# LongTarget/Fasim-LongTarget

Measured on AMD Instinct MI355X. Metric: SW Gcells/s (logical, whole job: stage 1+2+3 of the triplex scan), higher is better.
Workload: dtype u8

## Files before the change

### fasim-longtarget_amd/csrc/align.hip

```cpp
#include <hip/hip_runtime.h>
#include <stdint.h>
#include <stdlib.h>
#include "kernels.h"
#include "systolic.h"

namespace fasim {

constexpr int AL_SCALE = 32;
constexpr int AL_NEG = -32768;
constexpr int CODE_VOID = 4;
constexpr int CODE_SN = 5;
constexpr int TAG_LAST = 8;
constexpr int TAG_HZ = 16;
constexpr int FWD_KROW = 0x1FFFF;

__global__ void k_build_stream(const uint8_t* __restrict__ tcodes, const FwdProb* __restrict__ probs, int32_t nprob,
	uint8_t* __restrict__ stream, const uint32_t* __restrict__ zones)
{
	const int p = blockIdx.x;
	if (p >= nprob) return;
	const FwdProb pb = probs[p];
	uint8_t* s = stream + pb.stream_off;
	const uint32_t z = zones ? zones[p] : 0u;
	const int z1 = (int)(z & 0xffu), z2 = (int)((z >> 8) & 0xffu), z3 = (int)((z >> 16) & 0xffu);
// ... 490 lines not shown
			const int gp = in ? A.lo(k) : GL_NEG;
			const int ep = in ? A.hi(k) : GL_NEG;
			int e = max(ep - GAP_EXT, gp - GAP_OPEN);
			int g = diag > GL_NEG / 2 ? diag + swsc(q[read_end - i], tcode) : GL_NEG;
			g = max(g, max(e, F));
			const int rest = min(R - 1 - i, colrest);
			if (g <= 0 || g + 5 * rest < S) g = GL_NEG;
			if (e <= 0 || e + 5 * rest < S) e = GL_NEG;
			if (g == S) { *ref_begin = ref_end - j; *read_begin = read_end - i; return 0; }
			diag = gp;
			A.set(k, g, e);
			if (g > GL_NEG / 2 || e > GL_NEG / 2) { if (nlo < 0) nlo = i; nhi = i; }
			F = max(F - GAP_EXT, g - GAP_OPEN);
			if (F <= 0) F = GL_NEG;
			if (i > hi && F <= GL_NEG / 2 && diag <= GL_NEG / 2) break;
			if (i - lo + 2 >= FL_RING) return 2;
		}
		if (nlo < 0) return 1;
		lo = nlo; hi = nhi;
	}
	return 1;
}

template <int FL_WORDS, int FL_CELLS>
__global__ void __launch_bounds__(64) k_finish_lds(const uint8_t* __restrict__ tcodes, const uint8_t* __restrict__ qcodes,
	const FwdProb* __restrict__ probs, const FwdOut* __restrict__ fwd, const int32_t* __restrict__ order, int32_t nprob,
	uint8_t* __restrict__ dirs, AlignOutDev* __restrict__ out, uint32_t* __restrict__ cigar_pool, uint32_t pool_cap,
	uint32_t* __restrict__ pool_count)
{
	constexpr int FL_RING = FL_WORDS, FL_W = FL_WORDS / 2;
	__shared__ uint32_t lds[FL_WORDS * 64];
	const int gid = blockIdx.x * blockDim.x + threadIdx.x;
	if (gid >= nprob) return;
	const int pi = order ? order[gid] : gid;
	LdsArena A; A.base = lds + threadIdx.x;
	uint8_t* dir = dirs + (int64_t)blockIdx.x * (64 * FL_CELLS) + threadIdx.x;
	const FwdProb pb = probs[pi];
	const FwdOut fo = fwd[pi];
	AlignOutDev* o = out + pi;
	o->sw_score = 0; o->ref_begin = 0; o->ref_end = fo.ref_end; o->query_begin = 0; o->query_end = fo.read_end; o->cigar_len = 0;
	o->cigar_off = 0;
	if (fo.flags & 1) { o->status = 10; return; }
	if (fo.score <= 0 || fo.ref_end < 0) { o->status = 0; return; }
	const uint8_t* tw = tcodes + pb.tbase;
	int ref_begin = fo.ref_begin, read_begin = fo.read_begin;
	if (!(fo.flags & 2)) {
		if (fo.score >= 148 && fo.score < 255 - BIAS) { o->status = 11; return; }
		const int r = reverse_pass_lds<FL_RING>(tw, qcodes, fo.score, fo.ref_end, fo.read_end, A, &ref_begin, &read_begin);
		if (r) { o->status = r == 2 ? 2 : 11; return; }
	}
	o->ref_begin = ref_begin; o->query_begin = read_begin;
	const uint8_t* ref = tw + ref_begin;
	const uint8_t* read = qcodes + read_begin;
	const int refLen = fo.ref_end - ref_begin + 1, readLen = fo.read_end - read_begin + 1, score = fo.score;
	int band = (refLen > readLen ? refLen - readLen : readLen - refLen) + 1;
	int maxv = 0, width = 0, width_d = 0;
	do {
		width = band * 2 + 3; width_d = band * 2 + 1;
		if (width + 1 > FL_W || width_d * readLen > FL_CELLS) { o->status = 2; return; }
		for (int j = 1; j < width - 1; j++) A.set_lo(j, 0);
		for (int i = 0; i < readLen; i++) {
			int beg = 0, end = refLen - 1, u = 0;
			if (i - band > beg) beg = i - band;
			if (i + band < end) end = i + band;
			const int edge = end + 1 < width - 1 ? end + 1 : width - 1;
			int f = 0;
			A.set(0, 0, 0); A.set(edge, 0, 0); A.set_lo(FL_W, 0);
			const int x = i - band > 0 ? i - band : 0;
			const int xp = i - 1 - band > 0 ? i - 1 - band : 0;
			const int rd = read[i];
			const int rowcell = width_d * i;
			for (int j = beg; j <= end; j++) {
				u = j - x + 1;
				const int e = j - xp + 1, b = j - x, d = j - xp;
				int t1 = i == 0 ? -GAP_OPEN : A.lo(e) - GAP_OPEN;
				int t2 = i == 0 ? -GAP_EXT : A.hi(e) - GAP_EXT;
				const int ev = t1 > t2 ? t1 : t2;
				const int de = t1 > t2 ? 1 : 0;
				t1 = A.lo(FL_W + b) - GAP_OPEN;
				t2 = f - GAP_EXT;
				f = t1 > t2 ? t1 : t2;
				const int df = t1 > t2 ? 1 : 0;
				const int e1 = ev > 0 ? ev : 0;
				const int f1 = f > 0 ? f : 0;
				t1 = e1 > f1 ? e1 : f1;
				t2 = A.lo(d) + swsc(ref[j], rd);
				const int hv = t1 > t2 ? t1 : t2;
				A.set_hi(u, ev);
				A.set_lo(FL_W + u, hv);
				if (hv > maxv) maxv = hv;
				const int dh = (t1 <= t2) ? 0 : (e1 > f1 ? 1 : 2);
				dir[(int64_t)(rowcell + (j - x)) * 64] = (uint8_t)(de | (df << 1) | (dh << 2));
			}
			for (int j = 1; j <= u; j++) A.set_lo(j, A.lo(FL_W + j));
		}
		band *= 2;
		if (maxv < score && band > 4 * (refLen + readLen) + 16) { o->status = 3; return; }
	} while (maxv < score);
	band /= 2;
	uint32_t rc[ALIGN_MAX_CIGAR];
	int l = 0;
	int i = readLen - 1, j = refLen - 1, e = 0, state = 2, op = 0, prev_op = 0, status = 0;
	while (i > 0) {
		const int x = i - band > 0 ? i - band : 0;
		int beg = 0, end = refLen - 1;
		if (i - band > beg) beg = i - band;
		if (i + band < end) end = i + band;
		if (j < beg || j > end) { status = 3; break; }
		const uint32_t nib = dir[(int64_t)(width_d * i + (j - x)) * 64];
		int dv;
		const int dE = (nib & 1) ? 3 : 2, dF = (nib & 2) ? 5 : 4;
		if (state == 0) dv = dE; else if (state == 1) dv = dF; else { const int dh = (nib >> 2) & 3; dv = dh == 0 ? 1 : (dh == 1 ? dE : dF); }
		if (dv == 1) { --i; --j; state = 2; op = 0; }
		else if (dv == 2) { --i; state = 0; op = 1; }
		else if (dv == 3) { --i; state = 2; op = 1; }
		else if (dv == 4) { --j; state = 1; op = 2; }
		else { --j; state = 2; op = 2; }
		if (op == prev_op) ++e;
		else {
			if (l >= ALIGN_MAX_CIGAR) { status = 4; break; }
			rc[l++] = cig(e, prev_op);
			prev_op = op; e = 1;
		}
	}
	if (status == 0) {
		if (op == 0) { if (l >= ALIGN_MAX_CIGAR) status = 4; else rc[l++] = cig(e + 1, 0); }
		else { if (l + 2 > ALIGN_MAX_CIGAR) status = 4; else { rc[l++] = cig(e, op); rc[l++] = cig(1, 0); } }
	}
	if (status == 0) {
		const uint32_t off = atomicAdd(pool_count, (uint32_t)l);
		if ((uint64_t)off + (uint64_t)l > (uint64_t)pool_cap) status = 4;
		else { o->cigar_off = off; for (int k = 0; k < l; k++) cigar_pool[off + k] = rc[l - 1 - k]; }
	}
	o->status = status;
	if (status != 0) return;
	o->sw_score = score;
	o->cigar_len = l;
}

hipError_t launch_finish(const uint8_t* tcodes, const uint8_t* qcodes, const FwdProb* probs, const FwdOut* fwd, const int32_t* order,
	int32_t nprob, uint8_t* dirs, AlignOutDev* out, uint32_t* cigar_pool, uint32_t pool_cap, uint32_t* pool_count, hipStream_t st)
{
	if (nprob <= 0) return hipSuccess;
	hipError_t err = hipMemsetAsync(pool_count, 0, sizeof(uint32_t), st);
	if (err != hipSuccess) return err;
	hipLaunchKernelGGL((k_finish_lds<64, 2048>), dim3((nprob + 63) / 64), dim3(64), 0, st, tcodes, qcodes, probs, fwd, order, nprob, dirs, out,
		cigar_pool, pool_cap, pool_count);
	return hipGetLastError();
}

hipError_t launch_finish_mid(const uint8_t* tcodes, const uint8_t* qcodes, const FwdProb* probs, const FwdOut* fwd, const int32_t* idx_list,
	int32_t nlist, uint8_t* dirs, AlignOutDev* out, uint32_t* cigar_pool, uint32_t pool_cap, uint32_t* pool_count, hipStream_t st)
{
	if (nlist <= 0) return hipSuccess;
	static bool attr_set = false;
	if (!attr_set) { (void)hipFuncSetAttribute((const void*)k_finish_lds<256, 16384>, hipFuncAttributeMaxDynamicSharedMemorySize, 64 * 1024); attr_set = true; }
	hipLaunchKernelGGL((k_finish_lds<256, 16384>), dim3((nlist + 63) / 64), dim3(64), 0, st, tcodes, qcodes, probs, fwd, idx_list, nlist, dirs, out,
		cigar_pool, pool_cap, pool_count);
	return hipGetLastError();
}

hipError_t launch_finish_big(const uint8_t* tcodes, const uint8_t* qcodes, const FwdProb* probs, const FwdOut* fwd,
	const int32_t* idx_list, int32_t nlist, uint8_t* scratch, int32_t scratch_cap, AlignOutDev* out, uint32_t* cigar_pool,
	uint32_t pool_cap, uint32_t* pool_count, hipStream_t st)
{
	if (nlist <= 0) return hipSuccess;
	hipLaunchKernelGGL(k_finish, dim3((nlist + 63) / 64), dim3(64), 0, st, tcodes, qcodes, probs, fwd, nlist, scratch, scratch_cap, out,
		cigar_pool, pool_cap, pool_count, idx_list);
	return hipGetLastError();
}

}
```

### fasim-longtarget_amd/csrc/engine.cpp

```cpp
#include "engine.h"

extern "C" {

void fasim_params_default(fasim_params* p)
{
	p->rule = 0; p->cutLength = 5000; p->strand = 0; p->overlapLength = 100; p->ntMin = 20; p->ntMax = 100000;
	p->scoreMin = 0.0f; p->minIdentity = 60.0f; p->minStability = 1.0f; p->penaltyT = -1000; p->penaltyC = 0;
	p->cDistance = 15; p->cLength = 50; p->classicSim = 0;
}

const char* fasim_last_error(const fasim_engine* e) { return e ? e->err.c_str() : g_last_error.c_str(); }

int fasim_engine_create(int device, fasim_engine** out) { return fasim_engine_create_ex(device, 0, out); }

int fasim_engine_create_ex(int device, int32_t flags, fasim_engine** out)
{
	if (!out) return fail(nullptr, FASIM_E_ARG, "null out pointer");
	*out = nullptr;
	const bool tune = !(flags & FASIM_CREATE_NO_PROCESS_TUNING);
	if (tune) setenv("GPU_MAX_HW_QUEUES", "8", 0);
	if (tune) {
		static const bool once = [] {
			const char* e = getenv("FASIM_MALLOPT");
			if (e && atoi(e) == 0) return false;
// ... 25 lines not shown
	const char* env = getenv("FASIM_HOST_THREADS");
	E->host_threads = env ? std::max(1, atoi(env)) : (int)std::min(96u, std::max(1u, hc * 3 / 8));
	E->host_threads_total = E->host_threads;
	E->host_threads_explicit = env != nullptr;
	const char* v1 = getenv("FASIM_SCAN_V1");
	E->scan_v1 = v1 && atoi(v1) != 0;
	const char* a1 = getenv("FASIM_ALIGN_V1");
	E->align_v1 = a1 && atoi(a1) != 0;
	const char* sw = getenv("FASIM_STRIPED_WINDOW");
	E->striped_window = sw && atoi(sw) != 0;
	*out = E;
	return FASIM_OK;
}

void fasim_engine_destroy(fasim_engine* e)
{
	if (!e) return;
	for (fasim_engine* w : e->workers) fasim_engine_destroy(w);
	e->workers.clear();
	(void)hipSetDevice(e->device);
	DevBuf* bufs[] = { &e->q1, &e->q2, &e->enc_lut, &e->counter, &e->dna, &e->seg_start, &e->seg_len, &e->enc_ids, &e->tcodes,
		&e->colmax, &e->probs, &e->max_out, &e->unit_len, &e->stage1, &e->hits, &e->hits_total, &e->hit_off, &e->hit_cnt, &e->thr,
		&e->ends, &e->bprobs, &e->bout, &e->scratch, &e->dna_res, &e->colmax16, &e->unit_ids, &e->flags, &e->stage1_in, &e->hits2,
		&e->fprobs, &e->ftasks, &e->fstream, &e->fout, &e->aout, &e->cigpool, &e->cigcount, &e->forder, &e->scratch2, &e->boundary, &e->fboundary, &e->unit_hz,
		&e->unit_first, &e->hz_cols, &e->hz_plan, &e->hz_base, &e->hz_items, &e->snap, &e->hz_state, &e->hz_rows, &e->hz_chunk, &e->hz_src, &e->hz_zero,
		&e->qsim, &e->sim_min, &e->sim_row, &e->sim_ev, &e->sim_cnt, &e->sim_nodes,
		&e->ublk, &e->btarget, &e->bidx, &e->bcounts, &e->blist[0], &e->blist[1], &e->blist[2], &e->bslots[0], &e->bslots[1], &e->bslots[2],
		&e->bprev, &e->lane_ub, &e->fzones, &e->fubslot, &e->bdec, &e->btab, &e->swin, &e->unit_ovf, &e->track, &e->track_phase, &e->track_sat, &e->track_peaks, &e->sites_counts, &e->sites_offsets, &e->sites_runs, &e->sites_sat, &e->sa_q, &e->sa_tcodes, &e->sa_probs, &e->sa_ends, &e->sa_rows, &e->sa_items, &e->sa_dirs, &e->sa_cigar, &e->sa_ciglen,
		&e->rowmax16, &e->row_out, &e->row_gfirst, &e->row_sat, &e->oligo_q, &e->hist, &e->hist_zone, &e->hist_zones, &e->hist_sat,
		&e->vr_q, &e->vr_dna, &e->vr_alt, &e->vr_wins, &e->vr_probs, &e->vr_tcodes, &e->vr_rows, &e->vr_touch, &e->vr_out };
	for (auto& t : e->timed) { (void)hipEventDestroy(t.a); (void)hipEventDestroy(t.b); }
	for (hipEvent_t ev : e->ev_pool) (void)hipEventDestroy(ev);
	for (DevBuf* b : bufs) b->release();
	if (e->pin_dna) (void)hipHostFree(e->pin_dna);
	if (e->pin_sim) (void)hipHostFree(e->pin_sim);
	if (e->st) (void)hipStreamDestroy(e->st);
	delete e;
}

int fasim_set_option(fasim_engine* E, const char* key, int32_t value)
{
	if (!E || !key) return fail(E, FASIM_E_ARG, "null argument");
	if (!strcmp(key, "workers")) E->opt_workers = value > 0 ? value : 0;
	else if (!strcmp(key, "seg_batch")) E->opt_seg_batch = value > 0 ? value : 0;
	else if (!strcmp(key, "taper")) E->opt_taper = value;
	else if (!strcmp(key, "heavy_gate")) E->opt_gate = value;
	else if (!strcmp(key, "hazard_chunks")) E->hz_chunks = value;
	else if (!strcmp(key, "hazard_snapshots")) E->hz_snap = value;
	else if (!strcmp(key, "hazard_chunk_cols")) E->hz_target = value > 0 ? std::max(64, value) : 0;
	else if (!strcmp(key, "hazard_hot_weight")) E->hz_hot_w = value > 0 ? std::min(32, value) : 0;
	else if (!strcmp(key, "host_threads")) { if (value > 0) { E->host_threads = value; E->host_threads_total = value; E->host_threads_explicit = true; } }
	else if (!strcmp(key, "numa_affinity")) E->opt_numa = value != 0;
	else if (!strcmp(key, "band")) E->opt_band = value;
	else if (!strcmp(key, "dp_f16")) E->opt_dp_f16 = value;
	else if (!strcmp(key, "site_short")) E->opt_site_short = value;
	else if (!strcmp(key, "sim_lds")) E->opt_sim_lds = value < 0 ? -1 : value != 0;
	else if (!strcmp(key, "site_chunk")) E->opt_site_chunk = value > 0 ? value : 0;
	else if (!strcmp(key, "striped_window")) E->striped_window = value > 0;
	else return fail(E, FASIM_E_ARG, "unknown option %s", key);
	return FASIM_OK;
}

static int refuse_long_query(fasim_engine* E, int64_t len, int index)
{
	char which[32] = "";
	if (index >= 0) snprintf(which, sizeof which, " (query %d)", index);
	return fail(E, FASIM_E_UNSUPPORTED, "query of %lld nt%s exceeds the limit of %d nt: above it the reference's 16-bit stage-1 pass "
		"overruns its fixed workspace (stats.h:397) and its output is undefined", (long long)len, which, FASIM_MAX_QUERY);
}

int fasim_set_query(fasim_engine* E, const char* rna, int32_t len)
{
	if (!E) return fail(nullptr, FASIM_E_ARG, "null engine");
	if (!rna || len <= 0) return fail(E, FASIM_E_ARG, "empty query");
	if (len > FASIM_MAX_QUERY) return refuse_long_query(E, len, -1);
	HIPOK(hipSetDevice(E->device));
// ... 875 lines not shown
```

### fasim-longtarget_amd/csrc/engine.h

```cpp
#pragma once
#include <hip/hip_runtime.h>

#include <algorithm>
#include <atomic>
#include <chrono>
#include <sched.h>
#include <malloc.h>
#include <cstdarg>
#include <cstdio>
#include <cstdlib>
#include <cstring>
#include <deque>
#include <map>
#include <memory>
#include <string>
#include <condition_variable>
#include <mutex>
#include <thread>
#include <vector>

#include "../../include/fasim_hip.h"
#include "device_types.h"
#include "host_post.h"
#include "kernels.h"
// ... 28 lines not shown
	double t[N] = { 0 }; const char* name[N] = { nullptr };
	bool on = false;
	std::mutex mu;
	void add(int i, const char* nm, double dt) { if (on) { std::lock_guard<std::mutex> g(mu); t[i] += dt; name[i] = nm; } }
	void dump() { if (!on) return; for (int i = 0; i < N; i++) if (name[i]) fprintf(stderr, "[fasim prof] %-60s %12.6f\n", name[i], t[i]); }
	void reset() { for (int i = 0; i < N; i++) { t[i] = 0; name[i] = nullptr; } }
};
inline HostProf g_prof;
static inline double thread_cpu_s() { timespec ts; clock_gettime(CLOCK_THREAD_CPUTIME_ID, &ts); return (double)ts.tv_sec + 1e-9 * (double)ts.tv_nsec; }
struct CpuScope { int i; const char* nm; double t0; CpuScope(int i_, const char* n) : i(i_), nm(n), t0(g_prof.on ? thread_cpu_s() : 0.0) {} ~CpuScope() { if (g_prof.on) g_prof.add(i, nm, thread_cpu_s() - t0); } };
struct ProfScope { int i; const char* nm; double t0; ProfScope(int i_, const char* n) : i(i_), nm(n), t0(now_s()) {} ~ProfScope() { g_prof.add(i, nm, now_s() - t0); } };


struct fasim_engine {
	int device = 0;
	hipStream_t st = nullptr;
	std::string err;
	std::string rna;
	int m = 0;
	int snap_units = 0, snap_per_unit = 0;
	ScoreLut lut1, lut2;
	DevBuf q1, q2, enc_lut, counter, dna, seg_start, seg_len, enc_ids, tcodes, colmax, probs, max_out, unit_len,
		stage1, hits, hits_total, hit_off, hit_cnt, thr, ends, bprobs, bout, scratch, colmax16, unit_ids, flags, stage1_in, hits2,
		fprobs, ftasks, fstream, fout, aout, cigpool, cigcount, forder, scratch2, boundary, fboundary, unit_hz,
		unit_first, hz_cols, hz_plan, hz_base, hz_items, snap, hz_state, hz_rows, hz_chunk, hz_src, hz_zero,
		qsim, sim_min, sim_row, sim_ev, sim_cnt, sim_nodes,
		sim_req, sim_pairs, sim_used, sim_rounds, sim_col, sim_rowst, sim_state, sim_usedc, sim_debug, sim_nodes_in, sim_nodes_out, sim_out;
	bool align_v1 = false;
	std::vector<fasim_engine*> workers;
	struct HeavyGate { std::mutex m; std::condition_variable cv; int in_flight = 0; int cap = 3; };
	HeavyGate own_gate;
	HeavyGate* gate = nullptr;
	int host_threads_total = 1;
	int host_threads_share_total = 1;
	bool host_threads_explicit = false;
	int scan_workers = 1;
	std::atomic<int>* sim_in_flight = nullptr;
	std::atomic<int>* active_workers = nullptr;
	int sim_threads = 1;
	int opt_workers = 0, opt_seg_batch = 0;
	int opt_taper = -1, opt_gate = -1;
	int hz_chunks = -1, hz_snap = -1, hz_target = 0, hz_hot_w = 0;
	bool query_acgt = true;
	bool scan_v1 = false;
	int host_threads = 1;
	std::string dna_host;
	DevBuf dna_res;
	void* pin_dna = nullptr; size_t pin_cap = 0;
	void* pin_sim = nullptr; size_t pin_sim_cap = 0;
	struct Timed { hipEvent_t a, b; int family; };
	std::vector<Timed> timed;
	std::vector<hipEvent_t> ev_pool;
	double kernel_ms[FASIM_KERNEL_FAMILIES] = { 0 };
	int64_t kernel_launches[FASIM_KERNEL_FAMILIES] = { 0 };
	DevBuf ublk, btarget, bidx, bcounts, blist[3], bslots[3], bprev, lane_ub, fzones, fubslot, bdec, btab;
	int ublk_units = 0, ublk_blocks = 0;
	int opt_band = -1;
	int opt_dp_f16 = -1;
	DevBuf unit_ovf;
	DevBuf track, track_phase, track_sat;
	DevBuf track_peaks;
	DevBuf sites_counts, sites_offsets, sites_runs, sites_sat;
	DevBuf sa_q, sa_tcodes, sa_probs, sa_ends, sa_rows, sa_items, sa_dirs, sa_cigar, sa_ciglen;
	DevBuf hist, hist_zone, hist_zones, hist_sat;
	DevBuf vr_q, vr_dna, vr_alt, vr_wins, vr_probs, vr_tcodes, vr_rows, vr_touch, vr_out;
	int opt_sim_lds = -1;
	int opt_site_short = -1;
	int opt_site_chunk = 0;
	DevBuf oligo_q;
	DevBuf rowmax16, row_out, row_gfirst, row_sat;
	int opt_numa = 1;
	DevBuf swin;
	bool striped_window = false;
	int64_t sw_probs = 0;
	double sw_ms = 0.0;
};



inline int fail(fasim_engine* e, int code, const char* fmt, ...)
// ... 131 lines not shown
	if (sched_getaffinity(0, sizeof set, &set) == 0) { const int a = CPU_COUNT(&set); if (a > 0) n = std::min(n, a); }
	if (FILE* f = fopen("/sys/fs/cgroup/cpu.max", "r")) {
		char q[64] = { 0 }; long long period = 0;
		if (fscanf(f, "%63s %lld", q, &period) == 2 && strcmp(q, "max") != 0 && period > 0) { const long long c = atoll(q) / period; if (c >= 1) n = (int)std::min<long long>(n, c); }
		fclose(f);
	}
	return std::max(1, n);
}

inline int band_mode(const fasim_engine* E)
{
	static const int env = [] { const char* e = getenv("FASIM_BAND"); return e ? atoi(e) : 1; }();
	return E->opt_band >= 0 ? E->opt_band : env;
}
inline bool site_short_enabled(const fasim_engine* E)
{
	static const int env = [] { const char* e = getenv("FASIM_SITE_SHORT"); return e ? atoi(e) : 1; }();
	return (E->opt_site_short >= 0 ? E->opt_site_short : env) != 0;
}
inline bool dp_f16_mode(const fasim_engine* E)
{
	static const int env = [] { const char* e = getenv("FASIM_DP_F16"); return e ? atoi(e) : 1; }();
	return (E->opt_dp_f16 >= 0 ? E->opt_dp_f16 : env) != 0;
}
inline int band_mask(const fasim_engine* E)
{
	if (!band_mode(E) || E->align_v1 || E->scan_v1) return 0;
	return band_classes(E->m);
}

inline bool gpu_local_cpus(int device, cpu_set_t* out)
{
	char bus[64] = { 0 };
	if (hipDeviceGetPCIBusId(bus, (int)sizeof bus, device) != hipSuccess) { (void)hipGetLastError(); return false; }
	for (char* c = bus; *c; c++) if (*c >= 'A' && *c <= 'F') *c = (char)(*c - 'A' + 'a');
	char path[160]; snprintf(path, sizeof path, "/sys/bus/pci/devices/%s/local_cpulist", bus);
	FILE* f = fopen(path, "r");
	if (!f) return false;
	char list[1024] = { 0 };
	const bool ok = fgets(list, sizeof list, f) != nullptr;
	fclose(f);
	if (!ok) return false;
	cpu_set_t local; CPU_ZERO(&local);
	for (const char* p = list; *p && *p != '\n'; ) {
		char* e = nullptr;
		const long a = strtol(p, &e, 10);
// ... 203 lines not shown
```

### fasim-longtarget_amd/csrc/engine_scan.cpp

```cpp
#include "engine.h"
#include <memory>

int sim_forward_units(fasim_engine* E, const uint8_t* tcodes_dev, int tstride, const int32_t* unit_len_dev, const int32_t* unit_len_host,
	int first, int nrun, const int64_t* min_scores, std::atomic<int>* ready, std::vector<std::vector<fasim_sim_node>>& lists)
{
	static_assert(sizeof(SimNodeDev) == sizeof(fasim_sim_node) && SIM_K == FASIM_SIM_K, "node layout");
	if (nrun <= 0) return FASIM_OK;
	int maxlen = 1;
	for (int u = 0; u < nrun; u++) maxlen = std::max(maxlen, unit_len_host[first + u]);
	if (E->m > 65534 || maxlen > 65534) return fail(E, FASIM_E_UNSUPPORTED, "the SIM forward sweep holds start points in 16 bits: query %d / target %d nt is too long", E->m, maxlen);
	const int64_t row_stride = (maxlen + 2 + 15) & ~15;
	const uint32_t cap = (uint32_t)((maxlen + 15) & ~15);
	ProfScope fwd_wall(13, "-F forward sweep (k_sim_forward slices), wall");
	DevBuf& d_min = E->sim_min; DevBuf& d_row = E->sim_row; DevBuf& d_ev = E->sim_ev; DevBuf& d_cnt = E->sim_cnt; DevBuf& d_nodes = E->sim_nodes;
	int rc = upload(E, d_min, min_scores, sizeof(int64_t) * nrun); if (rc) return rc;
	int per_slice = 1024;
	{
		size_t free_b = 0, total_b = 0;
		const size_t unit_b = (size_t)64 * cap * sizeof(SimEvent) + (size_t)2 * row_stride * sizeof(uint64_t);
		if (hipMemGetInfo(&free_b, &total_b) == hipSuccess) {
			const size_t have = std::min<size_t>(((size_t)96 << 30) / (size_t)std::max(1, E->scan_workers), E->sim_ev.cap + free_b / 3);
			per_slice = (int)std::max<size_t>(256, std::min<size_t>(8192, have / unit_b));
		}
		const int nslices = (nrun + per_slice - 1) / per_slice;
// ... 631 lines not shown
				b0 += len;
			}
		}
		struct Item { int q; int64_t b0, b1; };
		std::vector<Item> items;
		items.reserve(chunks.size() * (size_t)nquery);
		for (int q = 0; q < nquery; q++) for (const auto& c : chunks) items.push_back({ q, c.first, c.second });
		nworkers = (int)std::min<size_t>((size_t)nworkers, items.size());
		while ((int)E->workers.size() < nworkers - 1) {
			fasim_engine* w = nullptr;
			int rc = fasim_engine_create(E->device, &w); if (rc) return fail(E, rc, "cannot create worker engine: %s", fasim_last_error(nullptr));
			E->workers.push_back(w);
		}
		std::atomic<int> active_workers(nworkers), sim_active(0);
		std::vector<fasim_engine*> ws(1, E);
		for (int k = 0; k < nworkers - 1; k++) ws.push_back(E->workers[k]);
		{
			const char* envg = getenv("FASIM_HEAVY_GATE");
			E->own_gate.cap = E->opt_gate >= 0 ? E->opt_gate : (envg ? atoi(envg) : 4);
		}
		for (fasim_engine* w : ws) {
			w->gate = (ws.size() > 1 && E->own_gate.cap > 0) ? &E->own_gate : nullptr;
			w->scan_v1 = E->scan_v1; w->align_v1 = E->align_v1; w->striped_window = E->striped_window;
			w->hz_chunks = E->hz_chunks; w->hz_snap = E->hz_snap; w->hz_target = E->hz_target; w->hz_hot_w = E->hz_hot_w; w->opt_band = E->opt_band; w->opt_dp_f16 = E->opt_dp_f16; w->opt_sim_lds = E->opt_sim_lds;
			w->host_threads = std::max(1, E->host_threads_total / nworkers);
			w->host_threads_share_total = E->host_threads_total; w->active_workers = &active_workers; w->sim_in_flight = &sim_active; w->scan_workers = (int)ws.size();
			{
				const int all = E->host_threads_explicit ? E->host_threads_total : usable_cores();
				w->sim_threads = std::max(1, all / (int)std::max<size_t>(1, std::min<size_t>((size_t)nworkers, items.size()) / 4));
			}
			HIPOK(hipSetDevice(E->device));
			int rc = upload(w, w->enc_ids, encs.data(), sizeof(int) * nenc); if (rc) return rc;
			drain_timed(w);
			for (int k = 0; k < FASIM_KERNEL_FAMILIES; k++) { w->kernel_ms[k] = 0; w->kernel_launches[k] = 0; }
			w->sw_probs = 0; w->sw_ms = 0.0;
		}
		std::vector<std::vector<RecPart>> per_item(items.size());
		std::vector<fasim_scan_stats> ist(items.size());
		for (auto& x : ist) memset(&x, 0, sizeof x);
		std::vector<double> it0(items.size(), 0.0), it1(items.size(), 0.0);
		std::vector<int> wrc(ws.size(), FASIM_OK);
		std::atomic<size_t> next(0);
		auto run = [&](size_t wi) {
			CpuScope cpu(28, "CPU seconds: worker threads themselves (HIP calls, lists, decisions)");
			(void)hipSetDevice(E->device);
			fasim_engine* w = ws[wi];
			for (;;) {
// ... 123 lines not shown
```

### fasim-longtarget_amd/csrc/engine_stage3.cpp

```cpp
#include "engine.h"


int run_finish(fasim_engine* E, const UnitBatch& B, const std::vector<WindowProb>& W, const std::vector<FwdOut>& fo,
	std::vector<AlignResult>& out, std::vector<uint32_t>& cigars, std::vector<char>& status, std::vector<int32_t>* path = nullptr);
bool align_v2_fits(const fasim_engine* E, const std::vector<WindowProb>& W);
static constexpr int CIGAR_LEN_ENDS_ONLY = -2;
int run_fwd(fasim_engine* E, const UnitBatch& B, const std::vector<WindowProb>& W, std::vector<FwdOut>& fo, bool word, const FwdZones* Z = nullptr);

int run_align(fasim_engine* E, const UnitBatch& B, const std::vector<WindowProb>& W, std::vector<AlignResult>& out,
	std::vector<uint32_t>& cigars, fasim_scan_stats* stats)
{
	const int n = (int)W.size();
	out.assign(n, AlignResult());
	if (!n) return FASIM_OK;
	ProfScope ps(6, "run_align (exact) total");
	std::vector<StripedProb> probs(n);
	for (int k = 0; k < n; k++) {
		probs[k].tbase = (int64_t)W[k].unit * B.tstride; probs[k].t0 = W[k].t0; probs[k].ref_len = W[k].len;
		probs[k].q_len = E->m; probs[k].unit = k; probs[k].aux = 0; probs[k].pad = 0;
	}
	HIPOK(E->ends.ensure(sizeof(AlignEnds) * n));
	int rc = run_striped(E, MODE_ALIGN, false, probs, false, tcv(E), E->m);
	if (rc) return rc;
	std::vector<AlignEnds> ends(n);
// ... 370 lines not shown
int run_finish(fasim_engine* E, const UnitBatch& B, const std::vector<WindowProb>& W, const std::vector<FwdOut>& fo,
	std::vector<AlignResult>& out, std::vector<uint32_t>& cigars, std::vector<char>& status, std::vector<int32_t>* path)
{
	const int n = (int)W.size();
	out.assign(n, AlignResult()); status.assign(n, 0);
	if (path) path->assign(n, 0);
	if (!n) return FASIM_OK;
	std::vector<char> tier(n, 0);
	auto settle = [&](const std::vector<AlignOutDev>& a, int pass) { for (int k = 0; k < n; k++) if (!tier[k] && a[k].status != 2) tier[k] = (char)pass; };
	ProfScope ps(4, "run_finish total");
	std::vector<FwdProb> probs(n);
	for (int k = 0; k < n; k++) { probs[k].tbase = (int64_t)W[k].unit * B.tstride + W[k].t0; probs[k].len = W[k].len; probs[k].stream_off = 0; }
	const int scratch_cap = 16384;
	int rc = upload_async(E, E->fprobs, probs.data(), sizeof(FwdProb) * n); if (rc) return rc;
	rc = upload_async(E, E->fout, fo.data(), sizeof(FwdOut) * n); if (rc) return rc;
	HIPOK(E->aout.ensure(sizeof(AlignOutDev) * n));
	const size_t pool_cap = (size_t)n * 12 + 4096;
	HIPOK(E->cigpool.ensure(pool_cap * sizeof(uint32_t)));
	HIPOK(E->cigcount.ensure(64));
	hipError_t he;
	std::vector<int32_t> order(n);
	{
		std::vector<int32_t> cnt(1026, 0);
		for (int k = 0; k < n; k++) cnt[std::min(1024, std::max(0, fo[k].score)) + 1]++;
		for (int b = 1; b < 1026; b++) cnt[b] += cnt[b - 1];
		for (int k = 0; k < n; k++) order[cnt[std::min(1024, std::max(0, fo[k].score))]++] = k;
		rc = upload_async(E, E->forder, order.data(), sizeof(int32_t) * n); if (rc) return rc;
	}
	HIPOK(E->scratch.ensure((size_t)((n + 63) / 64) * 64 * 2048));
	{ TimedScope ts(E, 3);
	he = launch_finish(tcv(E), E->q2.as<uint8_t>(), E->fprobs.as<FwdProb>(), E->fout.as<FwdOut>(),
		E->forder.as<int32_t>(), n, E->scratch.as<uint8_t>(), E->aout.as<AlignOutDev>(), E->cigpool.as<uint32_t>(), (uint32_t)pool_cap,
		E->cigcount.as<uint32_t>(), E->st); }
	if (he != hipSuccess) return fail(E, FASIM_E_HIP, "finish launch failed: %s", hipGetErrorString(he));
	std::vector<AlignOutDev> ao(n);
	uint32_t pool_used = 0;
	HIPOK(hipMemcpyAsync(ao.data(), E->aout.p, sizeof(AlignOutDev) * n, hipMemcpyDeviceToHost, E->st));
	HIPOK(hipMemcpyAsync(&pool_used, E->cigcount.p, sizeof pool_used, hipMemcpyDeviceToHost, E->st));
	HIPOK(hipStreamSynchronize(E->st));
	settle(ao, 1);
	{
		std::vector<int32_t> mid;
		for (int k = 0; k < n; k++) if (ao[k].status == 2) mid.push_back(k);
		if (!mid.empty()) {
			if (g_prof.on) g_prof.add(30, "finish: alignments sent to the 64 KB LDS pass (count)", 1e-6 * mid.size());
			rc = upload(E, E->unit_ids, mid.data(), sizeof(int32_t) * mid.size()); if (rc) return rc;
			HIPOK(E->scratch2.ensure((size_t)((mid.size() + 63) / 64) * 64 * 16384));
			{ TimedScope ts(E, 3);
			he = launch_finish_mid(tcv(E), E->q2.as<uint8_t>(), E->fprobs.as<FwdProb>(), E->fout.as<FwdOut>(), E->unit_ids.as<int32_t>(), (int)mid.size(),
				E->scratch2.as<uint8_t>(), E->aout.as<AlignOutDev>(), E->cigpool.as<uint32_t>(), (uint32_t)pool_cap, E->cigcount.as<uint32_t>(), E->st); }
			if (he != hipSuccess) return fail(E, FASIM_E_HIP, "finish (64 KB LDS) launch failed: %s", hipGetErrorString(he));
			HIPOK(hipMemcpyAsync(ao.data(), E->aout.p, sizeof(AlignOutDev) * n, hipMemcpyDeviceToHost, E->st));
			HIPOK(hipMemcpyAsync(&pool_used, E->cigcount.p, sizeof pool_used, hipMemcpyDeviceToHost, E->st));
			HIPOK(hipStreamSynchronize(E->st));
			settle(ao, 2);
		}
	}
	{
		const int caps[2] = { scratch_cap, 1 << 20 };
		for (int pass = 0; pass < 2; pass++) {
			std::vector<int32_t> big;
			for (int k = 0; k < n; k++) if (ao[k].status == 2) big.push_back(k);
			if (big.empty()) break;
			if (g_prof.on) g_prof.add(17 + pass, pass ? "finish: alignments sent to the 1 MB pass (count)" : "finish: alignments sent to the 16 KB pass (count)", 1e-6 * big.size());
			rc = upload(E, E->unit_ids, big.data(), sizeof(int32_t) * big.size()); if (rc) return rc;
			const size_t per_launch = std::max<size_t>(64, ((size_t)2 << 30) / (size_t)caps[pass]);
			HIPOK(E->scratch2.ensure(std::min(big.size(), per_launch) * (size_t)caps[pass]));
			for (size_t b0 = 0; b0 < big.size(); b0 += per_launch) {
				const size_t cnt = std::min(per_launch, big.size() - b0);
				{ TimedScope ts(E, 6);
				he = launch_finish_big(tcv(E), E->q2.as<uint8_t>(), E->fprobs.as<FwdProb>(), E->fout.as<FwdOut>(),
					E->unit_ids.as<int32_t>() + b0, (int)cnt, E->scratch2.as<uint8_t>(), caps[pass], E->aout.as<AlignOutDev>(),
					E->cigpool.as<uint32_t>(), (uint32_t)pool_cap, E->cigcount.as<uint32_t>(), E->st); }
// ... 307 lines not shown
```

### fasim-longtarget_amd/csrc/kernels.h

```cpp
#pragma once
#include <hip/hip_runtime.h>
#include <type_traits>
#include <vector>
#include "device_types.h"

namespace fasim {

enum StripedMode { MODE_PRE = 0, MODE_MAX1 = 1, MODE_ALIGN = 2, MODE_REV = 3 };

constexpr int HAZARD_MAX_CHUNKS = 512;
struct StripedLaunch {
	const uint8_t* tcodes;
	const uint8_t* qcodes;
	const StripedProb* probs;
	int32_t nprob;
	uint32_t* counter;
	ScoreLut lut;
	int32_t max_qlen;
	uint8_t* colmax;
	uint16_t* colmax_w = nullptr;
	int32_t* max_out;
	AlignEnds* ends;
	const uint16_t* state = nullptr; int32_t state_rows = 0; const int32_t* chunk_cols = nullptr; const int32_t* chunk_base = nullptr; uint8_t* chunk_rows = nullptr; int32_t row_stride = 0;
	int32_t* chunk_out = nullptr;
// ... 158 lines not shown
hipError_t launch_touch(const TouchLaunch& L, hipStream_t st);
hipError_t launch_touch_reduce(const TouchReduceLaunch& L, hipStream_t st);

struct RowFoldLaunch {
	const uint16_t* rowmax16;
	const int32_t* gfirst;
	int32_t ngroups, nenc, rows_total;
	TrackTable tab;
	uint16_t* out;
	uint8_t* sat;
};
hipError_t launch_rowfold(const RowFoldLaunch& L, hipStream_t st);

struct FwdLaunch {
	const uint8_t* stream; const FwdProb* probs; const int32_t* task_first; int32_t ntask; uint32_t* counter;
	const uint8_t* qcodes; int32_t m; FwdOut* out;
	uint4* boundary;
	int32_t word;
	uint16_t* lane_ub = nullptr; const int32_t* ub_slot = nullptr;
	int32_t f16 = 0;
};
hipError_t launch_build_stream(const uint8_t* tcodes, const FwdProb* probs, int32_t nprob, uint8_t* stream, const uint32_t* zones, hipStream_t st);
hipError_t launch_align_fwd(const FwdLaunch& L, hipStream_t st);
hipError_t launch_finish(const uint8_t* tcodes, const uint8_t* qcodes, const FwdProb* probs, const FwdOut* fwd, const int32_t* order,
	int32_t nprob, uint8_t* dirs, AlignOutDev* out, uint32_t* cigar_pool, uint32_t pool_cap, uint32_t* pool_count, hipStream_t st);

hipError_t launch_finish_mid(const uint8_t* tcodes, const uint8_t* qcodes, const FwdProb* probs, const FwdOut* fwd, const int32_t* idx_list,
	int32_t nlist, uint8_t* dirs, AlignOutDev* out, uint32_t* cigar_pool, uint32_t pool_cap, uint32_t* pool_count, hipStream_t st);
hipError_t launch_finish_big(const uint8_t* tcodes, const uint8_t* qcodes, const FwdProb* probs, const FwdOut* fwd,
	const int32_t* idx_list, int32_t nlist, uint8_t* scratch, int32_t scratch_cap, AlignOutDev* out, uint32_t* cigar_pool,
	uint32_t pool_cap, uint32_t* pool_count, hipStream_t st);

struct BandTry { int32_t prob, r0, theta_min, nq; };
constexpr int BAND_SLOT_COLS = 208;
constexpr int BAND_MAX_ZONES = 32;
constexpr int BAND_COUNT_COLS = 3 * BAND_MAX_ZONES, BAND_COUNT_HOT = BAND_COUNT_COLS + 3, BAND_COUNT_NOBAND = BAND_COUNT_COLS + 4, BAND_COUNTS = 128;
struct BandSelLaunch {
	const FwdProb* probs; const int32_t* target; const int32_t* idx; int32_t n, tstride;
	const uint16_t* ublk; int32_t ublk_blocks; int32_t m; const uint8_t* tcodes;
	const uint16_t* prev_ub = nullptr; const int32_t* prev = nullptr;
	BandTry* list[3]; uint16_t* slots[3]; uint32_t list_cap;
	int4* dec;
	uint32_t* counts;
	uint32_t* cursors;
	FwdOut* out; int32_t class_mask;
	int32_t debug = 0;
};
struct BandZoneTab { int32_t zbase, first, count, wg, nwg; };
struct BandLaunch { const BandTry* list; const uint16_t* slots; const BandZoneTab* tab; int32_t nwg, cls; const uint8_t* qcodes; int32_t m; FwdOut* out; };
int band_profile_lanes(int m);
int band_zone_stride(int m);
// ... 12 lines not shown
```

Baseline: 3212.

## Split finish kernel into reverse pass and band DP ordered by band work

Splits the per-lane finish kernel into a reverse-pass kernel that records the initial band width and a banded-DP kernel. Between them a device histogram, scan and scatter sorts problems by estimated band cells, so lanes in one wavefront do similar work. Problems whose band must grow are deferred to a second retry pass rather than iterating inside a divergent wavefront, and the host order now goes by descending score. This adds several small kernel launches, extra global traffic and an extra pass in exchange for less lane divergence.

```diff
diff --git a/fasim-longtarget_amd/csrc/align.hip b/fasim-longtarget_amd/csrc/align.hip
--- a/fasim-longtarget_amd/csrc/align.hip
+++ b/fasim-longtarget_amd/csrc/align.hip
@@ -536,24 +536,29 @@
 	return 1;
 }
 
-template <int FL_WORDS, int FL_CELLS>
-__global__ void __launch_bounds__(64) k_finish_lds(const uint8_t* __restrict__ tcodes, const uint8_t* __restrict__ qcodes,
+
+__device__ __forceinline__ int finish_bucket(int band, int readLen, int cells)
+{
+	const int key = max(0, min((2 * band + 1) * readLen, cells));
+	return FINISH_BUCKETS - 1 - key * FINISH_BUCKETS / (cells + 1);
+}
+
+template <int FL_RING>
+__global__ void __launch_bounds__(64) k_finish_rev(const uint8_t* __restrict__ tcodes, const uint8_t* __restrict__ qcodes,
 	const FwdProb* __restrict__ probs, const FwdOut* __restrict__ fwd, const int32_t* __restrict__ order, int32_t nprob,
-	uint8_t* __restrict__ dirs, AlignOutDev* __restrict__ out, uint32_t* __restrict__ cigar_pool, uint32_t pool_cap,
-	uint32_t* __restrict__ pool_count)
-{
-	constexpr int FL_RING = FL_WORDS, FL_W = FL_WORDS / 2;
-	__shared__ uint32_t lds[FL_WORDS * 64];
+	AlignOutDev* __restrict__ out, int32_t* __restrict__ bandw)
+{
+	__shared__ uint32_t lds[FL_RING * 64];
 	const int gid = blockIdx.x * blockDim.x + threadIdx.x;
 	if (gid >= nprob) return;
 	const int pi = order ? order[gid] : gid;
 	LdsArena A; A.base = lds + threadIdx.x;
-	uint8_t* dir = dirs + (int64_t)blockIdx.x * (64 * FL_CELLS) + threadIdx.x;
 	const FwdProb pb = probs[pi];
 	const FwdOut fo = fwd[pi];
 	AlignOutDev* o = out + pi;
 	o->sw_score = 0; o->ref_begin = 0; o->ref_end = fo.ref_end; o->query_begin = 0; o->query_end = fo.read_end; o->cigar_len = 0;
 	o->cigar_off = 0;
+	bandw[pi] = 0;
 	if (fo.flags & 1) { o->status = 10; return; }
 	if (fo.score <= 0 || fo.ref_end < 0) { o->status = 0; return; }
 	const uint8_t* tw = tcodes + pb.tbase;
@@ -564,10 +569,93 @@
 		if (r) { o->status = r == 2 ? 2 : 11; return; }
 	}
 	o->ref_begin = ref_begin; o->query_begin = read_begin;
-	const uint8_t* ref = tw + ref_begin;
+	o->status = 2;
+	const int refLen = fo.ref_end - ref_begin + 1, readLen = fo.read_end - read_begin + 1;
+	bandw[pi] = (refLen > readLen ? refLen - readLen : readLen - refLen) + 1;
+}
+
+constexpr int FINISH_SORT_THREADS = 1024;
+__global__ void __launch_bounds__(FINISH_SORT_THREADS) k_finish_count(const FwdOut* __restrict__ fwd, const AlignOutDev* __restrict__ out,
+	const int32_t* __restrict__ order, int32_t nprob, const int32_t* __restrict__ bandw, uint32_t* __restrict__ hist, int32_t cells)
+{
+	__shared__ uint32_t cnt[FINISH_BUCKETS];
+	const int t = threadIdx.x, gid = blockIdx.x * blockDim.x + t;
+	if (t < FINISH_BUCKETS) cnt[t] = 0;
+	__syncthreads();
+	if (gid < nprob) {
+		const int pi = order ? order[gid] : gid;
+		const int band = bandw[pi];
+		if (band > 0) atomicAdd(cnt + finish_bucket(band, fwd[pi].read_end - out[pi].query_begin + 1, cells), 1u);
+	}
+	__syncthreads();
+	if (t < FINISH_BUCKETS && cnt[t]) atomicAdd(hist + t, cnt[t]);
+}
+
+__global__ void __launch_bounds__(FINISH_BUCKETS) k_finish_scan(uint32_t* __restrict__ hist)
+{
+	__shared__ uint32_t s[FINISH_BUCKETS];
+	const int t = threadIdx.x;
+	const uint32_t v = hist[t];
+	s[t] = v;
+	__syncthreads();
+	for (int d = 1; d < FINISH_BUCKETS; d *= 2) {
+		const uint32_t a = t >= d ? s[t - d] : 0u;
+		__syncthreads();
+		s[t] += a;
+		__syncthreads();
+	}
+	hist[t] = s[t] - v;
+	if (t == FINISH_BUCKETS - 1) hist[FINISH_BUCKETS] = s[t];
+}
+
+__global__ void __launch_bounds__(FINISH_SORT_THREADS) k_finish_scatter(const FwdOut* __restrict__ fwd, const AlignOutDev* __restrict__ out,
+	const int32_t* __restrict__ order, int32_t nprob, const int32_t* __restrict__ bandw, uint32_t* __restrict__ hist, int32_t cells,
+	int32_t* __restrict__ sorted)
+{
+	__shared__ uint32_t cnt[FINISH_BUCKETS];
+	const int t = threadIdx.x, gid = blockIdx.x * blockDim.x + t;
+	if (t < FINISH_BUCKETS) cnt[t] = 0;
+	__syncthreads();
+	int pi = -1, bucket = 0;
+	uint32_t place = 0;
+	if (gid < nprob) {
+		const int p = order ? order[gid] : gid;
+		const int band = bandw[p];
+		if (band > 0) { pi = p; bucket = finish_bucket(band, fwd[p].read_end - out[p].query_begin + 1, cells); place = atomicAdd(cnt + bucket, 1u); }
+	}
+	__syncthreads();
+	if (t < FINISH_BUCKETS && cnt[t]) cnt[t] = atomicAdd(hist + t, cnt[t]);
+	__syncthreads();
+	if (pi >= 0) {
+		const uint32_t pos = cnt[bucket] + place;
+		if (pos < (uint32_t)nprob) sorted[pos] = pi;
+	}
+}
+
+template <int FL_WORDS, int FL_CELLS, bool RETRY>
+__global__ void __launch_bounds__(64) k_finish_band(const uint8_t* __restrict__ tcodes, const uint8_t* __restrict__ qcodes,
+	const FwdProb* __restrict__ probs, const FwdOut* __restrict__ fwd, const int32_t* __restrict__ list, const uint32_t* __restrict__ count,
+	int32_t nlist, uint8_t* __restrict__ dirs, AlignOutDev* __restrict__ out, uint32_t* __restrict__ cigar_pool, uint32_t pool_cap,
+	uint32_t* __restrict__ pool_count, int32_t* __restrict__ bandw)
+{
+	constexpr int FL_W = FL_WORDS / 2;
+	__shared__ uint32_t lds[FL_WORDS * 64];
+	const int gid = blockIdx.x * blockDim.x + threadIdx.x;
+	const int lim = count ? (int)min(*count, (uint32_t)nlist) : nlist;
+	if (gid >= lim) return;
+	const int pi = list ? list[gid] : gid;
+	int band = bandw[pi];
+	if (band <= 0) return;
+	if (!RETRY) bandw[pi] = 0;
+	LdsArena A; A.base = lds + threadIdx.x;
+	uint8_t* dir = dirs + (int64_t)blockIdx.x * (64 * FL_CELLS) + threadIdx.x;
+	const FwdProb pb = probs[pi];
+	const FwdOut fo = fwd[pi];
+	AlignOutDev* o = out + pi;
+	const int ref_begin = o->ref_begin, read_begin = o->query_begin;
+	const uint8_t* ref = tcodes + pb.tbase + ref_begin;
 	const uint8_t* read = qcodes + read_begin;
 	const int refLen = fo.ref_end - ref_begin + 1, readLen = fo.read_end - read_begin + 1, score = fo.score;
-	int band = (refLen > readLen ? refLen - readLen : readLen - refLen) + 1;
 	int maxv = 0, width = 0, width_d = 0;
 	do {
 		width = band * 2 + 3; width_d = band * 2 + 1;
@@ -610,6 +698,10 @@
 		}
 		band *= 2;
 		if (maxv < score && band > 4 * (refLen + readLen) + 16) { o->status = 3; return; }
+		if (!RETRY && maxv < score) {
+			bandw[pi] = band;
+			return;
+		}
 	} while (maxv < score);
 	band /= 2;
 	uint32_t rc[ALIGN_MAX_CIGAR];
@@ -652,26 +744,53 @@
 	o->cigar_len = l;
 }
 
+template <int FL_WORDS, int FL_CELLS, bool RETRY_LAUNCH>
+static hipError_t finish_pipeline(const uint8_t* tcodes, const uint8_t* qcodes, const FwdProb* probs, const FwdOut* fwd, const int32_t* list,
+	int32_t nlist, uint8_t* dirs, AlignOutDev* out, uint32_t* cigar_pool, uint32_t pool_cap, uint32_t* pool_count, const FinishSort& S, hipStream_t st)
+{
+	const dim3 grid((nlist + 63) / 64), block(64);
+	if (S.ordered) {
+		hipError_t err = hipMemsetAsync(S.hist, 0, sizeof(uint32_t) * 2 * (FINISH_BUCKETS + 1), st);
+		if (err != hipSuccess) return err;
+	}
+	if (FL_WORDS * 64 * 4 > 48 * 1024) {
+		(void)hipFuncSetAttribute((const void*)k_finish_rev<FL_WORDS>, hipFuncAttributeMaxDynamicSharedMemorySize, FL_WORDS * 64 * 4);
+		(void)hipFuncSetAttribute((const void*)k_finish_band<FL_WORDS, FL_CELLS, false>, hipFuncAttributeMaxDynamicSharedMemorySize, FL_WORDS * 64 * 4);
+		(void)hipFuncSetAttribute((const void*)k_finish_band<FL_WORDS, FL_CELLS, true>, hipFuncAttributeMaxDynamicSharedMemorySize, FL_WORDS * 64 * 4);
+	}
+	hipLaunchKernelGGL((k_finish_rev<FL_WORDS>), grid, block, 0, st, tcodes, qcodes, probs, fwd, list, nlist, out, S.bandw);
+	for (int pass = 0; pass < (RETRY_LAUNCH ? 2 : 1); pass++) {
+		uint32_t* hist = S.hist + pass * (FINISH_BUCKETS + 1);
+		if (S.ordered) {
+			const dim3 sgrid((nlist + FINISH_SORT_THREADS - 1) / FINISH_SORT_THREADS), sblock(FINISH_SORT_THREADS);
+			hipLaunchKernelGGL(k_finish_count, sgrid, sblock, 0, st, fwd, out, list, nlist, S.bandw, hist, FL_CELLS);
+			hipLaunchKernelGGL(k_finish_scan, dim3(1), dim3(FINISH_BUCKETS), 0, st, hist);
+			hipLaunchKernelGGL(k_finish_scatter, sgrid, sblock, 0, st, fwd, out, list, nlist, S.bandw, hist, FL_CELLS, S.sorted);
+		}
+		const int32_t* blist = S.ordered ? S.sorted : list;
+		const uint32_t* bcount = S.ordered ? hist + FINISH_BUCKETS : nullptr;
+		if (pass == 0 && RETRY_LAUNCH) hipLaunchKernelGGL((k_finish_band<FL_WORDS, FL_CELLS, false>), grid, block, 0, st, tcodes, qcodes, probs, fwd, blist, bcount, nlist, dirs,
+			out, cigar_pool, pool_cap, pool_count, S.bandw);
+		else hipLaunchKernelGGL((k_finish_band<FL_WORDS, FL_CELLS, true>), grid, block, 0, st, tcodes, qcodes, probs, fwd, blist, bcount, nlist, dirs,
+			out, cigar_pool, pool_cap, pool_count, S.bandw);
+	}
+	return hipGetLastError();
+}
+
 hipError_t launch_finish(const uint8_t* tcodes, const uint8_t* qcodes, const FwdProb* probs, const FwdOut* fwd, const int32_t* order,
-	int32_t nprob, uint8_t* dirs, AlignOutDev* out, uint32_t* cigar_pool, uint32_t pool_cap, uint32_t* pool_count, hipStream_t st)
+	int32_t nprob, uint8_t* dirs, AlignOutDev* out, uint32_t* cigar_pool, uint32_t pool_cap, uint32_t* pool_count, const FinishSort& S, hipStream_t st)
 {
 	if (nprob <= 0) return hipSuccess;
 	hipError_t err = hipMemsetAsync(pool_count, 0, sizeof(uint32_t), st);
 	if (err != hipSuccess) return err;
-	hipLaunchKernelGGL((k_finish_lds<64, 2048>), dim3((nprob + 63) / 64), dim3(64), 0, st, tcodes, qcodes, probs, fwd, order, nprob, dirs, out,
-		cigar_pool, pool_cap, pool_count);
-	return hipGetLastError();
+	return finish_pipeline<64, 2048, true>(tcodes, qcodes, probs, fwd, order, nprob, dirs, out, cigar_pool, pool_cap, pool_count, S, st);
 }
 
 hipError_t launch_finish_mid(const uint8_t* tcodes, const uint8_t* qcodes, const FwdProb* probs, const FwdOut* fwd, const int32_t* idx_list,
-	int32_t nlist, uint8_t* dirs, AlignOutDev* out, uint32_t* cigar_pool, uint32_t pool_cap, uint32_t* pool_count, hipStream_t st)
+	int32_t nlist, uint8_t* dirs, AlignOutDev* out, uint32_t* cigar_pool, uint32_t pool_cap, uint32_t* pool_count, const FinishSort& S, hipStream_t st)
 {
 	if (nlist <= 0) return hipSuccess;
-	static bool attr_set = false;
-	if (!attr_set) { (void)hipFuncSetAttribute((const void*)k_finish_lds<256, 16384>, hipFuncAttributeMaxDynamicSharedMemorySize, 64 * 1024); attr_set = true; }
-	hipLaunchKernelGGL((k_finish_lds<256, 16384>), dim3((nlist + 63) / 64), dim3(64), 0, st, tcodes, qcodes, probs, fwd, idx_list, nlist, dirs, out,
-		cigar_pool, pool_cap, pool_count);
-	return hipGetLastError();
+	return finish_pipeline<256, 16384, false>(tcodes, qcodes, probs, fwd, idx_list, nlist, dirs, out, cigar_pool, pool_cap, pool_count, S, st);
 }
 
 hipError_t launch_finish_big(const uint8_t* tcodes, const uint8_t* qcodes, const FwdProb* probs, const FwdOut* fwd,
diff --git a/fasim-longtarget_amd/csrc/engine.cpp b/fasim-longtarget_amd/csrc/engine.cpp
--- a/fasim-longtarget_amd/csrc/engine.cpp
+++ b/fasim-longtarget_amd/csrc/engine.cpp
@@ -71,7 +71,7 @@
 	DevBuf* bufs[] = { &e->q1, &e->q2, &e->enc_lut, &e->counter, &e->dna, &e->seg_start, &e->seg_len, &e->enc_ids, &e->tcodes,
 		&e->colmax, &e->probs, &e->max_out, &e->unit_len, &e->stage1, &e->hits, &e->hits_total, &e->hit_off, &e->hit_cnt, &e->thr,
 		&e->ends, &e->bprobs, &e->bout, &e->scratch, &e->dna_res, &e->colmax16, &e->unit_ids, &e->flags, &e->stage1_in, &e->hits2,
-		&e->fprobs, &e->ftasks, &e->fstream, &e->fout, &e->aout, &e->cigpool, &e->cigcount, &e->forder, &e->scratch2, &e->boundary, &e->fboundary, &e->unit_hz,
+		&e->fprobs, &e->ftasks, &e->fstream, &e->fout, &e->aout, &e->cigpool, &e->cigcount, &e->forder, &e->fsort, &e->scratch2, &e->boundary, &e->fboundary, &e->unit_hz,
 		&e->unit_first, &e->hz_cols, &e->hz_plan, &e->hz_base, &e->hz_items, &e->snap, &e->hz_state, &e->hz_rows, &e->hz_chunk, &e->hz_src, &e->hz_zero,
 		&e->qsim, &e->sim_min, &e->sim_row, &e->sim_ev, &e->sim_cnt, &e->sim_nodes,
 		&e->ublk, &e->btarget, &e->bidx, &e->bcounts, &e->blist[0], &e->blist[1], &e->blist[2], &e->bslots[0], &e->bslots[1], &e->bslots[2],
@@ -101,6 +101,7 @@
 	else if (!strcmp(key, "host_threads")) { if (value > 0) { E->host_threads = value; E->host_threads_total = value; E->host_threads_explicit = true; } }
 	else if (!strcmp(key, "numa_affinity")) E->opt_numa = value != 0;
 	else if (!strcmp(key, "band")) E->opt_band = value;
+	else if (!strcmp(key, "finish_order")) E->opt_finish_order = value;
 	else if (!strcmp(key, "dp_f16")) E->opt_dp_f16 = value;
 	else if (!strcmp(key, "site_short")) E->opt_site_short = value;
 	else if (!strcmp(key, "sim_lds")) E->opt_sim_lds = value < 0 ? -1 : value != 0;
diff --git a/fasim-longtarget_amd/csrc/engine.h b/fasim-longtarget_amd/csrc/engine.h
--- a/fasim-longtarget_amd/csrc/engine.h
+++ b/fasim-longtarget_amd/csrc/engine.h
@@ -74,7 +74,7 @@
 	ScoreLut lut1, lut2;
 	DevBuf q1, q2, enc_lut, counter, dna, seg_start, seg_len, enc_ids, tcodes, colmax, probs, max_out, unit_len,
 		stage1, hits, hits_total, hit_off, hit_cnt, thr, ends, bprobs, bout, scratch, colmax16, unit_ids, flags, stage1_in, hits2,
-		fprobs, ftasks, fstream, fout, aout, cigpool, cigcount, forder, scratch2, boundary, fboundary, unit_hz,
+		fprobs, ftasks, fstream, fout, aout, cigpool, cigcount, forder, fsort, scratch2, boundary, fboundary, unit_hz,
 		unit_first, hz_cols, hz_plan, hz_base, hz_items, snap, hz_state, hz_rows, hz_chunk, hz_src, hz_zero,
 		qsim, sim_min, sim_row, sim_ev, sim_cnt, sim_nodes,
 		sim_req, sim_pairs, sim_used, sim_rounds, sim_col, sim_rowst, sim_state, sim_usedc, sim_debug, sim_nodes_in, sim_nodes_out, sim_out;
@@ -108,6 +108,7 @@
 	DevBuf ublk, btarget, bidx, bcounts, blist[3], bslots[3], bprev, lane_ub, fzones, fubslot, bdec, btab;
 	int ublk_units = 0, ublk_blocks = 0;
 	int opt_band = -1;
+	int opt_finish_order = -1;
 	int opt_dp_f16 = -1;
 	DevBuf unit_ovf;
 	DevBuf track, track_phase, track_sat;
@@ -285,6 +286,11 @@
 {
 	static const int env = [] { const char* e = getenv("FASIM_DP_F16"); return e ? atoi(e) : 1; }();
 	return (E->opt_dp_f16 >= 0 ? E->opt_dp_f16 : env) != 0;
+}
+inline bool finish_ordered(const fasim_engine* E)
+{
+	static const int env = [] { const char* e = getenv("FASIM_FINISH_ORDER"); return e ? atoi(e) : 1; }();
+	return (E->opt_finish_order >= 0 ? E->opt_finish_order : env) != 0;
 }
 inline int band_mask(const fasim_engine* E)
 {
diff --git a/fasim-longtarget_amd/csrc/engine_scan.cpp b/fasim-longtarget_amd/csrc/engine_scan.cpp
--- a/fasim-longtarget_amd/csrc/engine_scan.cpp
+++ b/fasim-longtarget_amd/csrc/engine_scan.cpp
@@ -677,7 +677,7 @@
 		for (fasim_engine* w : ws) {
 			w->gate = (ws.size() > 1 && E->own_gate.cap > 0) ? &E->own_gate : nullptr;
 			w->scan_v1 = E->scan_v1; w->align_v1 = E->align_v1; w->striped_window = E->striped_window;
-			w->hz_chunks = E->hz_chunks; w->hz_snap = E->hz_snap; w->hz_target = E->hz_target; w->hz_hot_w = E->hz_hot_w; w->opt_band = E->opt_band; w->opt_dp_f16 = E->opt_dp_f16; w->opt_sim_lds = E->opt_sim_lds;
+			w->hz_chunks = E->hz_chunks; w->hz_snap = E->hz_snap; w->hz_target = E->hz_target; w->hz_hot_w = E->hz_hot_w; w->opt_band = E->opt_band; w->opt_finish_order = E->opt_finish_order; w->opt_dp_f16 = E->opt_dp_f16; w->opt_sim_lds = E->opt_sim_lds;
 			w->host_threads = std::max(1, E->host_threads_total / nworkers);
 			w->host_threads_share_total = E->host_threads_total; w->active_workers = &active_workers; w->sim_in_flight = &sim_active; w->scan_workers = (int)ws.size();
 			{
diff --git a/fasim-longtarget_amd/csrc/engine_stage3.cpp b/fasim-longtarget_amd/csrc/engine_stage3.cpp
--- a/fasim-longtarget_amd/csrc/engine_stage3.cpp
+++ b/fasim-longtarget_amd/csrc/engine_stage3.cpp
@@ -416,16 +416,21 @@
 	std::vector<int32_t> order(n);
 	{
 		std::vector<int32_t> cnt(1026, 0);
-		for (int k = 0; k < n; k++) cnt[std::min(1024, std::max(0, fo[k].score)) + 1]++;
+		for (int k = 0; k < n; k++) cnt[1024 - std::min(1024, std::max(0, fo[k].score)) + 1]++;
 		for (int b = 1; b < 1026; b++) cnt[b] += cnt[b - 1];
-		for (int k = 0; k < n; k++) order[cnt[std::min(1024, std::max(0, fo[k].score))]++] = k;
+		for (int k = 0; k < n; k++) order[cnt[1024 - std::min(1024, std::max(0, fo[k].score))]++] = k;
 		rc = upload_async(E, E->forder, order.data(), sizeof(int32_t) * n); if (rc) return rc;
 	}
 	HIPOK(E->scratch.ensure((size_t)((n + 63) / 64) * 64 * 2048));
+	const size_t hist_bytes = sizeof(uint32_t) * 2 * (FINISH_BUCKETS + 1);
+	HIPOK(E->fsort.ensure(hist_bytes + sizeof(int32_t) * 2 * (size_t)n));
+	FinishSort fs;
+	fs.hist = E->fsort.as<uint32_t>(); fs.bandw = reinterpret_cast<int32_t*>(fs.hist + 2 * (FINISH_BUCKETS + 1)); fs.sorted = fs.bandw + n;
+	fs.ordered = finish_ordered(E) ? 1 : 0;
 	{ TimedScope ts(E, 3);
 	he = launch_finish(tcv(E), E->q2.as<uint8_t>(), E->fprobs.as<FwdProb>(), E->fout.as<FwdOut>(),
 		E->forder.as<int32_t>(), n, E->scratch.as<uint8_t>(), E->aout.as<AlignOutDev>(), E->cigpool.as<uint32_t>(), (uint32_t)pool_cap,
-		E->cigcount.as<uint32_t>(), E->st); }
+		E->cigcount.as<uint32_t>(), fs, E->st); }
 	if (he != hipSuccess) return fail(E, FASIM_E_HIP, "finish launch failed: %s", hipGetErrorString(he));
 	std::vector<AlignOutDev> ao(n);
 	uint32_t pool_used = 0;
@@ -442,7 +447,7 @@
 			HIPOK(E->scratch2.ensure((size_t)((mid.size() + 63) / 64) * 64 * 16384));
 			{ TimedScope ts(E, 3);
 			he = launch_finish_mid(tcv(E), E->q2.as<uint8_t>(), E->fprobs.as<FwdProb>(), E->fout.as<FwdOut>(), E->unit_ids.as<int32_t>(), (int)mid.size(),
-				E->scratch2.as<uint8_t>(), E->aout.as<AlignOutDev>(), E->cigpool.as<uint32_t>(), (uint32_t)pool_cap, E->cigcount.as<uint32_t>(), E->st); }
+				E->scratch2.as<uint8_t>(), E->aout.as<AlignOutDev>(), E->cigpool.as<uint32_t>(), (uint32_t)pool_cap, E->cigcount.as<uint32_t>(), fs, E->st); }
 			if (he != hipSuccess) return fail(E, FASIM_E_HIP, "finish (64 KB LDS) launch failed: %s", hipGetErrorString(he));
 			HIPOK(hipMemcpyAsync(ao.data(), E->aout.p, sizeof(AlignOutDev) * n, hipMemcpyDeviceToHost, E->st));
 			HIPOK(hipMemcpyAsync(&pool_used, E->cigcount.p, sizeof pool_used, hipMemcpyDeviceToHost, E->st));
diff --git a/fasim-longtarget_amd/csrc/kernels.h b/fasim-longtarget_amd/csrc/kernels.h
--- a/fasim-longtarget_amd/csrc/kernels.h
+++ b/fasim-longtarget_amd/csrc/kernels.h
@@ -204,11 +204,18 @@
 };
 hipError_t launch_build_stream(const uint8_t* tcodes, const FwdProb* probs, int32_t nprob, uint8_t* stream, const uint32_t* zones, hipStream_t st);
 hipError_t launch_align_fwd(const FwdLaunch& L, hipStream_t st);
+constexpr int FINISH_BUCKETS = 256;
+struct FinishSort {
+	int32_t* bandw;
+	int32_t* sorted;
+	uint32_t* hist;
+	int32_t ordered;
+};
 hipError_t launch_finish(const uint8_t* tcodes, const uint8_t* qcodes, const FwdProb* probs, const FwdOut* fwd, const int32_t* order,
-	int32_t nprob, uint8_t* dirs, AlignOutDev* out, uint32_t* cigar_pool, uint32_t pool_cap, uint32_t* pool_count, hipStream_t st);
+	int32_t nprob, uint8_t* dirs, AlignOutDev* out, uint32_t* cigar_pool, uint32_t pool_cap, uint32_t* pool_count, const FinishSort& S, hipStream_t st);
 
 hipError_t launch_finish_mid(const uint8_t* tcodes, const uint8_t* qcodes, const FwdProb* probs, const FwdOut* fwd, const int32_t* idx_list,
-	int32_t nlist, uint8_t* dirs, AlignOutDev* out, uint32_t* cigar_pool, uint32_t pool_cap, uint32_t* pool_count, hipStream_t st);
+	int32_t nlist, uint8_t* dirs, AlignOutDev* out, uint32_t* cigar_pool, uint32_t pool_cap, uint32_t* pool_count, const FinishSort& S, hipStream_t st);
 hipError_t launch_finish_big(const uint8_t* tcodes, const uint8_t* qcodes, const FwdProb* probs, const FwdOut* fwd,
 	const int32_t* idx_list, int32_t nlist, uint8_t* scratch, int32_t scratch_cap, AlignOutDev* out, uint32_t* cigar_pool,
 	uint32_t pool_cap, uint32_t* pool_count, hipStream_t st);
```

Result: no change. 3227, median of 3 (+0.5%).
